# matteocarnelos/microflow-rs

Measured on AMD Instinct MI355X. Metric: inferences/sec (int8) for person_detect.tflite, higher is better.
Workload: dtype i8; 1 GPU; person_detect.tflite batch=65536 per GPU, predict_inner int8->int8, inputs resident in HBM; per_gpu_batch=65536, global_batch=65536, parallelism=batch shard x1, no data-path collective

## Files before the change

microflow_rs_amd/csrc/k_quad.hip:

```cpp
#include "k_common.hpp"

#include <algorithm>
#include <type_traits>

#ifndef MF_QUAD_PRIO
#define MF_QUAD_PRIO 1
#endif
#ifndef MF_Q13_X2A
#define MF_Q13_X2A 0
#define MF_Q13_X2B 0
#define MF_Q57_X2A 3
#define MF_Q57_X2B 3
#endif

#ifndef MF_QUAD_ASM_LDS
#define MF_QUAD_ASM_LDS 0
#endif
#ifndef MF_QUAD_ASM_CLOBBER
#define MF_QUAD_ASM_CLOBBER 1
#endif
#ifndef MF_QUAD_STEM_LDS
#define MF_QUAD_STEM_LDS 1
#endif
#ifndef MF_QUAD_CNT_WAIT
#define MF_QUAD_CNT_WAIT 1
#endif
#ifndef MF_RR_SPARSE
#define MF_RR_SPARSE 0
#endif
#ifndef MF_RR_BLOCK
#define MF_RR_BLOCK 1
#endif
#ifndef MF_RR_SP_PAD
#define MF_RR_SP_PAD 7
#endif
#ifndef MF_Q57_DB
#define MF_Q57_DB 0
#endif
#ifndef MF_QUAD_KO
#define MF_QUAD_KO 0
#endif

namespace mf {
namespace k {
typedef float f32x4 __attribute__((ext_vector_type(4)));

__device__ __forceinline__ void lds_store_asm(uint8_t *p, int off, uint2 v) {
    typedef unsigned int u32x2_ __attribute__((ext_vector_type(2)));
    const uint32_t a = (uint32_t)(uintptr_t)(lds_u8_t *)p;
    const u32x2_ d = {v.x, v.y};
#if MF_QUAD_ASM_CLOBBER
    asm volatile("ds_write_b64 %0, %1 offset:%2" : : "v"(a), "v"(d), "i"(off) : "memory");
#else
    asm volatile("ds_write_b64 %0, %1 offset:%2" : : "v"(a), "v"(d), "i"(off));
#endif
}
__device__ __forceinline__ void lds_store_asm(uint8_t *p, int off, uint4 v) {
    const uint32_t a = (uint32_t)(uintptr_t)(lds_u8_t *)p;
    const u32x4 d = {v.x, v.y, v.z, v.w};
#if MF_QUAD_ASM_CLOBBER
    asm volatile("ds_write_b128 %0, %1 offset:%2" : : "v"(a), "v"(d), "i"(off) : "memory");
#else
    asm volatile("ds_write_b128 %0, %1 offset:%2" : : "v"(a), "v"(d), "i"(off));
#endif
}
template <bool ASMST> __device__ __forceinline__ void quad_barrier() {
    if constexpr (ASMST) asm volatile("s_waitcnt lgkmcnt(0)" ::: "memory");
    wg_sync();
}
__device__ __forceinline__ void quad_barrier_raw() {
    mf_jitter();
    asm volatile("s_waitcnt lgkmcnt(0)\n\ts_barrier" ::: "memory");
    mf_jitter();
}

template <int H_, int W_, int C_, int S_, int N_, int CG_, int CY_, int ORD_, int ROWPAD_, int TS_>
struct RrGeom {
    static constexpr int H = H_, W = W_, C = C_, S = S_, N = N_, CG = CG_, CY = CY_, ORD = ORD_, ROWPAD = ROWPAD_, TS = TS_;
    static constexpr bool PAIR = C == 8;
    static constexpr int OH = (H + S - 1) / S, OW = (W + S - 1) / S, OWC = PAIR ? OW / 2 : OW;
    static constexpr int NQ = PAIR ? 1 : C / 16, CX = 16 / (CG * CY);
    static constexpr int LP = C < 16 ? 16 : C;
    static constexpr int ROWB = W * C, ROW = LP + ROWB + LP + ROWPAD, TILE = (H + 2) * ROW;
    static constexpr int IMG = H * ROWB, ROWCH = ROWB / 16, OPIX = OH * OW;
    static constexpr int NT = (PAIR ? 2 * N : N) / 16, LB = 4 * NT;
    static_assert(C == 8 || C == 16 || C == 32, "register-resident pairs: C <= 32");
    static_assert(CG * CY * CX == 16 && OH % CY == 0 && OWC % CX == 0, "column grid");
    static_assert(ROWB % 16 == 0 && ROWCH <= 64 && ROW % 16 == 0, "staging geometry");
    static_assert(!PAIR || (S == 1 && OW % 2 == 0), "pair columns");
    static_assert(LB == 8 || LB == 16, "one 8- or 16-byte store per lane");
};

template <typename T> struct DstTile {
    static constexpr int TILE = T::TILE, ROW = T::ROW, C = T::C;
};
template <> struct DstTile<void> {
    static constexpr int TILE = 0, ROW = 0, C = 0;
};

template <typename Ge, int G, int NACT, int MG, uint32_t XR4, int X2 = 0>
struct RrPhase {
    static constexpr int NWAVE = NACT;
    static constexpr int UG = G / Ge::CG, UY = Ge::OH / Ge::CY, UX = Ge::OWC / Ge::CX;
    static constexpr int PSY = cgcd(UY, NWAVE), PSX = cgcd(UX, NWAVE / PSY), PSG = cgcd(UG, NWAVE / PSY / PSX);
    static_assert(G % Ge::CG == 0 && PSY * PSX * PSG == NWAVE, "the unit grid does not divide over the waves");
    static constexpr int NUG = UG / PSG, NUY = UY / PSY, NUX = UX / PSX, NU = NUG * NUY * NUX;
    static constexpr int T_UG = Ge::CG * Ge::TILE, T_UY = Ge::CY * Ge::S * Ge::ROW, T_UX = Ge::PAIR ? Ge::CX * 16 : Ge::CX * Ge::S * Ge::C;
    static constexpr int NQ = Ge::NQ, NT = Ge::NT;

    static constexpr bool SP = MF_RR_SPARSE == 1 || (MF_RR_SPARSE == 2 && !Ge::PAIR) || (MF_RR_SPARSE == 3 && Ge::PAIR);
    int tbase[NQ];
    v4i Adw[NQ][3];
    int tb0[NQ], tb1[NQ], tb9[NQ];
    v4i As[NQ];
    int Ai[NQ];
    long A9[NQ];
    float4 dA[NQ], dS[NQ];
    int4 dK[NQ];
    long Apw[NT];
    float4 cA[NT], cS[NT];
    int4 cK[NT];
    int dst_lane;
    int cg, wug;
    float dlo, dhi, plo, phi;

    template <typename NEXT>
    __device__ __forceinline__ void init(const DwPwArgs &p, int lane, int wave) {
        const int col = lane & 15, g = lane >> 4;
        int cy, cx;
        {
            constexpr int ORD = Ge::ORD, CGc = Ge::CG, CYc = Ge::CY, CXc = Ge::CX;
            constexpr int D0 = (ORD == 0 || ORD == 1) ? CGc : (ORD == 2 || ORD == 3) ? CYc : CXc;
            constexpr int D1 = (ORD == 2 || ORD == 4) ? CGc : (ORD == 0 || ORD == 5) ? CYc : CXc;
            const int i0 = col % D0, i1 = (col / D0) % D1, i2 = col / (D0 * D1);
            cg = (ORD == 0 || ORD == 1) ? i0 : (ORD == 2 || ORD == 4) ? i1 : i2;
            cy = (ORD == 2 || ORD == 3) ? i0 : (ORD == 0 || ORD == 5) ? i1 : i2;
            cx = (ORD == 4 || ORD == 5) ? i0 : (ORD == 1 || ORD == 3) ? i1 : i2;
        }
        const int wpy = wave % PSY, wpx = (wave / PSY) % PSX, wpg = wave / (PSY * PSX);
        wug = wpg * Ge::CG;
        const int wave_t = wpg * T_UG + wpy * T_UY + wpx * T_UX;
        auto chunk_addr = [&](int q, int ty, int gch) {
            if constexpr (Ge::PAIR) {
                return cg * Ge::TILE + (cy + ty) * Ge::ROW + Ge::LP + (2 * cx - 2) * 8 + gch * 16 + wave_t;
            } else {
                const int xl = cx * Ge::S + gch - 1;
                return cg * Ge::TILE + (cy * Ge::S + ty) * Ge::ROW + Ge::LP + xl * Ge::C + 16 * (q ^ tile_swz<Ge::TS>(xl)) + wave_t;
            }
        };
#pragma unroll
        for (int q = 0; q < NQ; ++q) {
            tbase[q] = chunk_addr(q, 0, g);
            tb0[q] = g < 3 ? chunk_addr(q, 0, g) : chunk_addr(q, 1, 0);
            tb1[q] = g < 2 ? chunk_addr(q, 1, g + 1) : chunk_addr(q, 2, g - 2);
            tb9[q] = chunk_addr(q, 2, 2) + 8 * (g & 1);
        }
        const int opar = Ge::PAIR ? (g >> 1) : 0;
        const int n0 = Ge::PAIR ? 8 * (g & 1) : (Ge::N / 4) * g;
        const int ox = (Ge::PAIR ? 2 * cx + opar : cx) + wpx * (Ge::PAIR ? 2 : 1) * Ge::CX;
        const int oy = cy + wpy * Ge::CY;
        if constexpr (std::is_void<NEXT>::value) {
            dst_lane = ((cg + wug) * Ge::OPIX + oy * Ge::OW + ox) * Ge::N + n0;
        } else {
            static_assert(NEXT::H == Ge::OH && NEXT::W == Ge::OW && NEXT::C == Ge::N, "the next pair consumes this pair's output");
            static_assert(tile_swz<NEXT::TS>(((Ge::PAIR ? 2 : 1) * Ge::CX) * 255) == 0 || NEXT::TS == 0, "x step vs swizzle");
            const int chunk = n0 >> 4, within = n0 & 15;
            dst_lane = (cg + wug) * NEXT::TILE + (oy + 1) * NEXT::ROW + NEXT::LP + ox * NEXT::C +
                       16 * (NEXT::NQ > 1 ? (chunk ^ tile_swz<NEXT::TS>(ox)) : chunk) + within;
        }
#pragma unroll
        for (int q = 0; q < NQ; ++q) {
            if constexpr (SP) {
                const v4i w0 = ((const v4i *)p.dw.wsp)[(q * 64 + lane) * 2], w1 = ((const v4i *)p.dw.wsp)[(q * 64 + lane) * 2 + 1];
                As[q] = w0, Ai[q] = w1[0];
                A9[q] = (long)(((unsigned long)(uint32_t)w1[2] << 32) | (unsigned long)(uint32_t)w1[1]);
            } else {
#pragma unroll
                for (int ty = 0; ty < 3; ++ty) Adw[q][ty] = ((const v4i *)p.dw.wmm)[(q * 3 + ty) * 64 + lane];
            }
            const int ch4 = Ge::PAIR ? (g & 1) : 4 * q + g;
            dA[q] = ((const float4 *)p.dw.A)[ch4];
            dS[q] = ((const float4 *)p.dw.S)[ch4];
            dK[q] = magic4<MG>(((const int4 *)p.dw.Kc)[ch4]);
        }
#pragma unroll
        for (int m = 0; m < NT; ++m) {
            Apw[m] = ((const long *)p.pw.wrr)[m * 64 + lane];
            cA[m] = *(const float4 *)(p.pw.A + n0 + 4 * m);
            cS[m] = *(const float4 *)(p.pw.S + n0 + 4 * m);
            cK[m] = magic4<MG>(*(const int4 *)(p.pw.Kc + n0 + 4 * m));
        }
        dlo = p.dw.lo_f, dhi = p.dw.hi_f, plo = p.pw.lo_f, phi = p.pw.hi_f;
    }

    template <typename NEXT, bool ASMST = false>
    __device__ __forceinline__ void run(const uint8_t *tb, uint8_t *dst, int gvalid) const {
        constexpr bool TO_LDS = !std::is_void<NEXT>::value;
        constexpr int XF = Ge::PAIR ? 2 : 1;
        constexpr int D_UG = TO_LDS ? Ge::CG * DstTile<NEXT>::TILE : Ge::CG * Ge::OPIX * Ge::N;
        constexpr int D_UY = TO_LDS ? Ge::CY * DstTile<NEXT>::ROW : Ge::CY * Ge::OW * Ge::N;
        constexpr int D_UX = TO_LDS ? XF * Ge::CX * DstTile<NEXT>::C : XF * Ge::CX * Ge::N;
#ifdef MF_QUAD_UB
        constexpr int UB = NU % MF_QUAD_UB == 0 ? MF_QUAD_UB : 1;
#else
        constexpr int UB = NQ > 1 ? 1 : (NU % 2 == 0 ? 2 : 1);
#endif
        auto coords = [](int iu, int &ug, int &uy, int &ux) constexpr {
            ug = (iu / (NUY * NUX)) * PSG, uy = ((iu / NUX) % NUY) * PSY, ux = (iu % NUX) * PSX;
        };
        auto toff_of = [&](int iu) constexpr {
            int ug = 0, uy = 0, ux = 0;
            coords(iu, ug, uy, ux);
            return ug * T_UG + uy * T_UY + ux * T_UX;
        };
        v4i bq[UB][NQ][3], bn[UB][NQ][3];
        long b9[UB][NQ], n9[UB][NQ];
        auto load_taps = [&](v4i (&b)[3], long &e, int q, int toff) {
            if constexpr (SP) {
                b[0] = *(const v4i *)(tb + tb0[q] + toff), b[1] = *(const v4i *)(tb + tb1[q] + toff);
                e = *(const long *)(tb + tb9[q] + toff);
            } else {
#pragma unroll
                for (int ty = 0; ty < 3; ++ty) b[ty] = ((MF_QUAD_KO & 32) && ty > 0) ? b[0] : *(const v4i *)(tb + tbase[q] + toff + ty * Ge::ROW);
            }
        };
#pragma unroll
        for (int u = 0; u < UB; ++u)
#pragma unroll
            for (int q = 0; q < NQ; ++q) load_taps(bq[u][q], b9[u][q], q, toff_of(u));
#pragma unroll
        for (int t0 = 0; t0 < NU; t0 += UB) {
            v4i acc[UB][NQ];
#pragma unroll
            for (int u = 0; u < UB; ++u)
#pragma unroll
                for (int q = 0; q < NQ; ++q) acc[u][q] = v4i{dK[q].x, dK[q].y, dK[q].z, dK[q].w};
#if MF_QUAD_PRIO
            __builtin_amdgcn_s_setprio(MF_QUAD_PRIO);
#endif
            if constexpr (SP) {
                typedef int v8i_ __attribute__((ext_vector_type(8)));
#pragma unroll
                for (int u = 0; u < UB; ++u)
#pragma unroll
                    for (int q = 0; q < NQ; ++q) acc[u][q] = __builtin_amdgcn_mfma_i32_16x16x32_i8(A9[q], b9[u][q], acc[u][q], 0, 0, 0);
                if (t0 + UB < NU) {
#pragma unroll
                    for (int u = 0; u < UB; ++u)
#pragma unroll
                        for (int q = 0; q < NQ; ++q) load_taps(bn[u][q], n9[u][q], q, toff_of(t0 + UB + u));
                }
#pragma unroll
                for (int u = 0; u < UB; ++u)
#pragma unroll
                    for (int q = 0; q < NQ; ++q) {
#if MF_RR_SP_PAD == 11
                        asm volatile("s_nop 11" : "+v"(acc[u][q]));
#else
                        asm volatile("s_nop 7" : "+v"(acc[u][q]));
#endif
                    }
#pragma unroll
                for (int u = 0; u < UB; ++u)
#pragma unroll
                    for (int q = 0; q < NQ; ++q) {
                        const v4i &lo = bq[u][q][0], &hi = bq[u][q][1];
                        const v8i_ B = {lo[0], lo[1], lo[2], lo[3], hi[0], hi[1], hi[2], hi[3]};
                        acc[u][q] = __builtin_amdgcn_smfmac_i32_16x16x128_i8(As[q], B, acc[u][q], Ai[q], 0, 0);
                    }
            } else {
#pragma unroll
                for (int ty = 0; ty < ((MF_QUAD_KO & 256) ? 2 : 3); ++ty)
#pragma unroll
                    for (int u = 0; u < UB; ++u)
#pragma unroll
                        for (int q = 0; q < NQ; ++q)
                            acc[u][q] = __builtin_amdgcn_mfma_i32_16x16x64_i8(Adw[q][ty], bq[u][q][ty], acc[u][q], 0, 0, 0);
            }
#if MF_QUAD_PRIO
            __builtin_amdgcn_s_setprio(0);
#endif
            if (!SP && t0 + UB < NU) {
#pragma unroll
                for (int u = 0; u < UB; ++u)
#pragma unroll
                    for (int q = 0; q < NQ; ++q) load_taps(bn[u][q], n9[u][q], q, toff_of(t0 + UB + u));
            }
#pragma unroll
            for (int u = 0; u < UB; ++u) {
                uint32_t d[2] = {0u, 0u};
                if constexpr ((MF_QUAD_KO & 1) != 0) {
#pragma unroll
                    for (int q = 0; q < NQ; ++q) d[q] = (uint32_t)(acc[u][q][0] ^ acc[u][q][1] ^ acc[u][q][2] ^ acc[u][q][3]);
                } else if constexpr (NQ == 2 && (X2 & 1) != 0) {
                    requant_pack4x2<MG, XR4>(acc[u][0], dA[0], dS[0], acc[u][1], dA[1], dS[1], dlo, dhi, d[0], d[1]);
                } else {
#pragma unroll
                    for (int q = 0; q < NQ; ++q)
                        d[q] = requant_pack4<MG, XR4>(acc[u][q][0], acc[u][q][1], acc[u][q][2], acc[u][q][3], dA[q], dS[q], dlo, dhi);
                }
                const long bop = (long)(((unsigned long)d[1] << 32) | (unsigned long)d[0]);
                uint32_t packed[NT];
                if constexpr ((MF_QUAD_KO & 2) != 0) {
#pragma unroll
                    for (int m = 0; m < NT; ++m) {
                        v4i pa = {cK[m].x, cK[m].y, cK[m].z, cK[m].w};
                        pa = __builtin_amdgcn_mfma_i32_16x16x32_i8(Apw[m], bop, pa, 0, 0, 0);
                        packed[m] = (uint32_t)(pa[0] ^ pa[1] ^ pa[2] ^ pa[3]);
                    }
                } else if constexpr ((X2 & 2) != 0) {
                    static_assert((X2 & 2) == 0 || NT % 2 == 0, "pointwise tiles in pairs");
#pragma unroll
                    for (int m = 0; m < NT; m += 2) {
                        v4i pa = {cK[m].x, cK[m].y, cK[m].z, cK[m].w}, pb2 = {cK[m + 1].x, cK[m + 1].y, cK[m + 1].z, cK[m + 1].w};
                        pa = __builtin_amdgcn_mfma_i32_16x16x32_i8(Apw[m], bop, pa, 0, 0, 0);
                        pb2 = __builtin_amdgcn_mfma_i32_16x16x32_i8(Apw[m + 1], bop, pb2, 0, 0, 0);
                        requant_pack4x2<MG, XR4>(pa, cA[m], cS[m], pb2, cA[m + 1], cS[m + 1], plo, phi, packed[m], packed[m + 1]);
                    }
                } else {
#pragma unroll
                    for (int m = 0; m < NT; ++m) {
                        v4i pa = {cK[m].x, cK[m].y, cK[m].z, cK[m].w};
                        pa = __builtin_amdgcn_mfma_i32_16x16x32_i8(Apw[m], bop, pa, 0, 0, 0);
                        packed[m] = requant_pack4<MG, XR4>(pa[0], pa[1], pa[2], pa[3], cA[m], cS[m], plo, phi);
                    }
                }
                int ug = 0, uy = 0, ux = 0;
                coords(t0 + u, ug, uy, ux);
                const int doff = ug * D_UG + uy * D_UY + ux * D_UX;
                if (G == 1 || cg + wug + ug * Ge::CG < gvalid) {
                    if constexpr (TO_LDS && ASMST) {
                        static_assert(G * DstTile<NEXT>::TILE < 65536, "tile offsets fit the ds offset field");
                        if constexpr (Ge::LB == 8) lds_store_asm(dst + dst_lane, doff, make_uint2(packed[0], packed[1]));
                        else lds_store_asm(dst + dst_lane, doff, make_uint4(packed[0], packed[1], packed[2], packed[3]));
                    } else if constexpr (TO_LDS) {
                        if constexpr (Ge::LB == 8) *(uint2 *)(dst + dst_lane + doff) = make_uint2(packed[0], packed[1]);
                        else *(uint4 *)(dst + dst_lane + doff) = make_uint4(packed[0], packed[1], packed[2], packed[3]);
                    } else if (!(MF_QUAD_KO & 4) || packed[0] == 0x12345678u) {
                        if constexpr (Ge::LB == 8) st_out(dst + dst_lane + doff, make_uint2(packed[0], packed[1]));
                        else st_out(dst + dst_lane + doff, make_uint4(packed[0], packed[1], packed[2], packed[3]));
                    }
                }
            }
#pragma unroll
            for (int u = 0; u < UB; ++u)
#pragma unroll
                for (int q = 0; q < NQ; ++q) {
#pragma unroll
                    for (int ty = 0; ty < 3; ++ty) bq[u][q][ty] = bn[u][q][ty];
                    b9[u][q] = n9[u][q];
                }
        }
    }
};

template <typename Ge, int NWAVE_, int MG, uint32_t XR4>
struct BlkPhase {
    static constexpr int NWAVE = NWAVE_, NU = Ge::W / 16;
    static constexpr int LP = 4, ROW = 320, PLANE = (Ge::H + 2) * ROW, BYTES = 2 * PLANE;
    static_assert(Ge::C == 8 && Ge::S == 1 && Ge::N == 16 && Ge::CG == 1, "block form: 8 -> 16 channels, stride 1, one image per step");
    static_assert(Ge::H == 4 * NWAVE && Ge::W % 16 == 0, "two block rows per wave, whole units per row");
    static_assert(ROW >= 4 * Ge::W + 2 * LP && ROW % 256 == 64 && BYTES % 16 == 0 && PLANE + 64 * NU + 8 < 65536, "tile A planes");
    int tbase;
    int dst_lane;
    v4i Adw[2];
    long Apw[4];
    float4 dA[2], dS[2], cA, cS;
    int4 dK[2], cK;
    float dlo, dhi, plo, phi;

    template <typename NEXT>
    __device__ __forceinline__ void init(const DwPwArgs &p, int lane, int wave) {
        static_assert(NEXT::H == Ge::OH && NEXT::W == Ge::OW && NEXT::C == Ge::N && NEXT::NQ == 1, "pair B consumes this pair's output, unswizzled");
        const int n = lane & 15, g = lane >> 4, by = 2 * wave + (n >> 3), bcx = n & 7;
        tbase = (2 * by + g) * ROW + 8 * bcx;
        dst_lane = (2 * by + 1) * NEXT::ROW + NEXT::LP + 32 * bcx + 4 * g;
#pragma unroll
        for (int q = 0; q < 2; ++q) {
            Adw[q] = ((const v4i *)p.dw.wblk)[q * 64 + lane];
            dA[q] = ((const float4 *)p.dw.A)[q];
            dS[q] = ((const float4 *)p.dw.S)[q];
            dK[q] = magic4<MG>(((const int4 *)p.dw.Kc)[q]);
        }
#pragma unroll
        for (int s = 0; s < 4; ++s) Apw[s] = ((const long *)p.pw.wiso)[s * 64 + lane];
        cA = *(const float4 *)(p.pw.A + 4 * g);
        cS = *(const float4 *)(p.pw.S + 4 * g);
        cK = magic4<MG>(*(const int4 *)(p.pw.Kc + 4 * g));
        dlo = p.dw.lo_f, dhi = p.dw.hi_f, plo = p.pw.lo_f, phi = p.pw.hi_f;
    }

    template <typename NEXT, bool ASMST = false>
    __device__ __forceinline__ void run(const uint8_t *tb, uint8_t *dst, int) const {
        static_assert(!ASMST, "the block form stores with plain LDS stores");
        typedef unsigned int u32x2_ __attribute__((ext_vector_type(2)));
        typedef __attribute__((address_space(3))) const volatile u32x2_ lds_cv2;
        v4i b[NU][2];
#pragma unroll
        for (int u = 0; u < NU; ++u)
#pragma unroll
            for (int q = 0; q < 2; ++q) {
                lds_u8_t *a = (lds_u8_t *)(tb + tbase) + (q * PLANE + 64 * u);
                const u32x2_ lo = *(lds_cv2 *)a, hi = *(lds_cv2 *)(a + 8);
                b[u][q] = v4i{(int)lo[0], (int)lo[1], (int)hi[0], (int)hi[1]};
            }
#pragma unroll
        for (int u = 0; u < NU; ++u) {
            v4i acc[2];
#if MF_QUAD_PRIO
            __builtin_amdgcn_s_setprio(MF_QUAD_PRIO);
#endif
#pragma unroll
            for (int q = 0; q < 2; ++q)
                acc[q] = __builtin_amdgcn_mfma_i32_16x16x64_i8(Adw[q], b[u][q], v4i{dK[q].x, dK[q].y, dK[q].z, dK[q].w}, 0, 0, 0);
#if MF_QUAD_PRIO
            __builtin_amdgcn_s_setprio(0);
#endif
            uint32_t d[2];
#pragma unroll
            for (int q = 0; q < 2; ++q) d[q] = requant_pack4<MG, XR4>(acc[q][0], acc[q][1], acc[q][2], acc[q][3], dA[q], dS[q], dlo, dhi);
            const long bop = (long)(((unsigned long)d[1] << 32) | (unsigned long)d[0]);
#pragma unroll
            for (int s = 0; s < 4; ++s) {
                const v4i pa = __builtin_amdgcn_mfma_i32_16x16x32_i8(Apw[s], bop, v4i{cK.x, cK.y, cK.z, cK.w}, 0, 0, 0);
                *(uint32_t *)(dst + dst_lane + 256 * u + (s >> 1) * NEXT::ROW + (s & 1) * 16) =
                    requant_pack4<MG, XR4>(pa[0], pa[1], pa[2], pa[3], cA, cS, plo, phi);
            }
        }
    }
};


#ifndef MF_Q13B_ROWPAD
#define MF_Q13B_ROWPAD 32
#endif
#ifndef MF_Q13A_ROWPAD
#define MF_Q13A_ROWPAD 32
#endif
struct Quad13 {
    using A = RrGeom<48, 48, 8, 1, 16, 1, 4, 0, MF_Q13A_ROWPAD, 0x000>;
    using B = RrGeom<48, 48, 16, 2, 32, 1, 2, 0, MF_Q13B_ROWPAD, 0x000>;
    static constexpr int G = 1, NTHR = 768, WPE = 3, ACT_A = 12, ACT_B = 12, X2A = MF_Q13_X2A, X2B = MF_Q13_X2B;
    static constexpr bool DBA = false;
    static constexpr const char *name = "quad_rr<48,48,8,1,16|48,48,16,2,32>";
};
struct Quad57 {
    using A = RrGeom<24, 24, 32, 1, 32, 1, 2, 0, 0, 0x002>;
    using B = RrGeom<24, 24, 32, 2, 64, 1, 4, 0, 32, 0x002>;
    static constexpr int G = 1, NTHR = 256, WPE = 2, ACT_A = 4, ACT_B = 3, X2A = MF_Q57_X2A, X2B = MF_Q57_X2B;
    static constexpr bool DBA = MF_Q57_DB != 0;
    static constexpr const char *name = "quad_rr<24,24,32,1,32|24,24,32,2,64>";
};



template <typename P, typename = void> struct blk_or {
    static constexpr int ROW = 0, LP = 0, PLANE = 0;
};
template <typename P> struct blk_or<P, std::void_t<decltype(P::PLANE)>> {
    static constexpr int ROW = P::ROW, LP = P::LP, PLANE = P::PLANE;
};
template <typename Q, bool STEM> constexpr bool quad_blk() {
    return STEM && MF_RR_BLOCK != 0 && MF_QUAD_ASM_LDS == 0;
}
template <typename Q, bool STEM, int MG, uint32_t XR4>
using QuadPhaseA = std::conditional_t<quad_blk<Q, STEM>(), BlkPhase<typename Q::A, Q::ACT_A, MG, XR4>, RrPhase<typename Q::A, Q::G, Q::ACT_A, MG, XR4, Q::X2A>>;
template <typename Q, bool STEM> constexpr int quad_buf_a() {
    if constexpr (quad_blk<Q, STEM>()) return BlkPhase<typename Q::A, Q::ACT_A, 1, 0u>::BYTES;
    else return Q::G * Q::A::TILE;
}
template <typename Q, bool STEM> constexpr int quad_stem_bytes() {
    return STEM ? 16 + (2 * Q::A::H + 2) * (2 * Q::A::W) : 0;
}
template <typename Q, bool STEM, int MG, uint32_t XR4, bool F32IN = false>
__global__ __launch_bounds__(Q::NTHR, Q::WPE) void quad_rr(const int8_t *__restrict__ in, int8_t *__restrict__ out, QuadArgs p, int batch) {
    static_assert(!F32IN || STEM, "the f32 entry is the stem's");
    using GA = typename Q::A;
    using GB = typename Q::B;
    epi_enter<MG>();
    constexpr int G = Q::G, NTHR = Q::NTHR, NWAVE = NTHR / 64;
    constexpr bool DBA = Q::DBA && !STEM;
    constexpr bool BLK = quad_blk<Q, STEM>();
    constexpr int BUF_A = quad_buf_a<Q, STEM>(), OFF_B = (DBA ? 2 : 1) * BUF_A + 512, BUF_B = G * GB::TILE, OFF_S = OFF_B + BUF_B + 512;
    constexpr int S_GUARD = 16, SW = 2 * GA::W, SH = 2 * GA::H, S_TILE = quad_stem_bytes<Q, STEM>(), OFF_Q = OFF_S + S_TILE;
    constexpr int OFF_F = OFF_Q + 16;
    constexpr int OFF_C = OFF_F + (F32IN ? 4 * SH * SW : 0);
    constexpr bool ASMST = MF_QUAD_ASM_LDS == 2 || (MF_QUAD_ASM_LDS == 1 && STEM);
    constexpr bool STEM_LDS = STEM && MF_QUAD_STEM_LDS != 0 && ((!F32IN && MG == 3) || MF_QUAD_STEM_LDS > 1);
    static_assert(!STEM || (G == 1 && GA::C == 8 && GA::W == 48 && (GA::H / 2) % NWAVE == 0 && (SH * SW) % 1024 == 0 && S_TILE % 16 == 0),
                  "stem phase: 8 channels, 24 pixel pairs per output row, whole row pairs per wave");
    extern __shared__ __attribute__((aligned(16))) uint8_t lds[];
    const int tid = threadIdx.x, lane = tid & 63;
    const int wave = __builtin_amdgcn_readfirstlane(tid >> 6);
    DynSteps dq;
    dq.init(lds + OFF_Q, p.a.dw.queue, tid, p.a.dw.qcfg);
    if constexpr (STEM)
        for (int i = tid; i < S_TILE / 16; i += NTHR) ((uint4 *)(lds + OFF_S))[i] = make_uint4(p.stem_izp4, p.stem_izp4, p.stem_izp4, p.stem_izp4);
    if constexpr (STEM_LDS)
        if (tid < 152) ((uint32_t *)(lds + OFF_C))[tid] = p.stem[tid] + ((MG != 0 && tid >= 144) ? (uint32_t)MF_MAGIC_I : 0u);
    for (int i = tid; i < OFF_B / 16; i += NTHR) ((uint4 *)lds)[i] = make_uint4(p.a.dw.izp4, p.a.dw.izp4, p.a.dw.izp4, p.a.dw.izp4);
    for (int i = tid; i < (BUF_B + 512) / 16; i += NTHR) ((uint4 *)(lds + OFF_B))[i] = make_uint4(p.b.dw.izp4, p.b.dw.izp4, p.b.dw.izp4, p.b.dw.izp4);
    QuadPhaseA<Q, STEM, MG, XR4> pa;
    RrPhase<GB, G, Q::ACT_B, MG, XR4, Q::X2B> pb;
    pa.template init<GB>(p.a, lane, wave);
    pb.template init<void>(p.b, lane, wave);
    wg_sync();

    auto stage = [&](int st, int buf = 0) {
        if constexpr (F32IN) {
            constexpr int NI = SH * SW * 4 / 1024;
            static_assert(NI % NWAVE == 0, "f32 staging: whole pieces per wave");
#pragma unroll
            for (int k = 0; k < NI / NWAVE; ++k) {
                const int r = k * NWAVE + wave;
                dma16(in + ((size_t)st * (SH * SW * 4) + r * 1024 + lane * 16), lds + OFF_F + r * 1024);
            }
            return;
        }
        if constexpr (STEM) {
            constexpr int NI = SH * SW / 1024;
#pragma unroll
            for (int k = 0; k < (NI + NWAVE - 1) / NWAVE; ++k) {
                const int r = k * NWAVE + wave;
                if (r < NI) dma16(in + ((size_t)st * (SH * SW) + r * 1024 + lane * 16), lds + OFF_S + S_GUARD + SW + r * 1024);
            }
            return;
        }
        constexpr int NROWS = G * GA::H;
        const int src_lane = GA::NQ > 1 ? (lane ^ tile_swz<GA::TS>(lane / (GA::NQ > 1 ? GA::NQ : 1))) : lane;
#pragma unroll
        for (int k = 0; k < (NROWS + NWAVE - 1) / NWAVE; ++k) {
            const int r = k * NWAVE + wave;
            const int gi = r / GA::H, y = r % GA::H;
            if (r < NROWS && st * G + gi < batch && lane < GA::ROWCH)
                dma16(in + ((size_t)(st * G + gi) * GA::IMG + y * GA::ROWB + src_lane * 16), lds + buf * BUF_A + gi * GA::TILE + (y + 1) * GA::ROW + GA::LP);
        }
    };
    auto quant_rows = [&]() {
        if constexpr (F32IN && !(MF_QUAD_KO & 64)) {
            constexpr int RPW = GA::H / 2 / NWAVE, NR = 4 * RPW + 1, C4 = SW / 4, NIT = (NR * C4 + 63) / 64;
            asm volatile("" ::: "memory");
            if constexpr (MG == 3) __builtin_amdgcn_s_setreg(0x801, 0);
            asm volatile("" ::: "memory");
            const int y0 = 4 * RPW * wave - 1;
#pragma unroll
            for (int it = 0; it < NIT; ++it) {
                const int item = it * 64 + lane, row = item / C4, c4 = item - row * C4, y = y0 + row;
                if (item < NR * C4 && y >= 0) {
                    const f32x4 v = *(const f32x4 *)(lds + OFF_F + (y * SW + 4 * c4) * 4);
                    int qv[4];
                    float q[4];
                    bool plain = p.in_fast != 0;
#pragma unroll
                    for (int e = 0; e < 4; ++e) {
                        const float q0 = __fmul_rn(v[e], p.in_rcp);
                        q[e] = __fmaf_rn(__fmaf_rn(-p.in_scale, q0, v[e]), p.in_rcp, q0);
                        plain = plain && (__builtin_fabsf(q[e]) <= 3.0e38f);
                    }
                    if constexpr ((MF_QUAD_KO & 128) != 0) {
#pragma unroll
                        for (int e = 0; e < 4; ++e) qv[e] = __float_as_int(v[e]);
                    } else if (__builtin_expect(plain, 1)) {
#pragma unroll
                        for (int e = 0; e < 4; ++e) {
                            const float t = __fadd_rn(q[e], p.in_zp_f);
                            const float r = __fadd_rn(t, __builtin_copysignf(0x1.fffffep-2f, t));
                            qv[e] = (int)__builtin_amdgcn_fmed3f(r, p.in_sat_lo, p.in_sat_hi);
                        }
                    } else {
#pragma unroll
                        for (int e = 0; e < 4; ++e) {
                            const float t = __fadd_rn(__fdiv_rn(v[e], p.in_scale), p.in_zp_f);
                            const float r = __fadd_rn(t, __builtin_copysignf(0x1.fffffep-2f, t));
                            qv[e] = (r != r) ? 0 : (int)__builtin_amdgcn_fmed3f(r, p.in_sat_lo, p.in_sat_hi);
                        }
                    }
                    *(uint32_t *)(lds + OFF_S + S_GUARD + (y + 1) * SW + 4 * c4) = pack4(qv[0], qv[1], qv[2], qv[3]) ^ p.in_xr4;
                }
            }
            asm volatile("" ::: "memory");
            if constexpr (MG == 3) __builtin_amdgcn_s_setreg(0x801, 3);
            asm volatile("" ::: "memory");
        }
    };
    auto stem_phase = [&](const uint32_t *sc) {
        constexpr int RPW = GA::H / 2 / NWAVE;
        const int col = lane & 15, g = lane >> 4;
        const int cq = (g & 1) * 4;
        long Aw;
        v4i cA_, cS_, cK;
        if constexpr (STEM_LDS) {
            const uint32_t *lsc = (const uint32_t *)(lds + OFF_C);
            Aw = *(const long *)(lsc + 2 * lane);
            cA_ = *(const v4i *)(lsc + 128 + cq), cS_ = *(const v4i *)(lsc + 136 + cq), cK = *(const v4i *)(lsc + 144 + cq);
        } else {
            typedef __attribute__((address_space(1))) const uint32_t g_u32;
            g_u32 *gsc = (g_u32 *)(uintptr_t)sc;
            typedef long i64x1 __attribute__((ext_vector_type(1)));
            Aw = (*(__attribute__((address_space(1))) const i64x1 *)(gsc + 2 * lane))[0];
            cA_ = *(__attribute__((address_space(1))) const v4i *)(gsc + 128 + cq), cS_ = *(__attribute__((address_space(1))) const v4i *)(gsc + 136 + cq);
            const v4i ck_ = *(__attribute__((address_space(1))) const v4i *)(gsc + 144 + cq);
            const int4 ck = magic4<MG>(make_int4(ck_[0], ck_[1], ck_[2], ck_[3]));
            cK = v4i{ck.x, ck.y, ck.z, ck.w};
        }
        const float4 cA = make_float4(__int_as_float(cA_[0]), __int_as_float(cA_[1]), __int_as_float(cA_[2]), __int_as_float(cA_[3]));
        const float4 cS = make_float4(__int_as_float(cS_[0]), __int_as_float(cS_[1]), __int_as_float(cS_[2]), __int_as_float(cS_[3]));
        const int oy1 = col >= 8 ? 1 : 0, j1 = col >= 8 ? col - 8 : 16 + col;
        const int off0 = S_GUARD + g * SW + 4 * col - 4, off1 = S_GUARD + (2 * oy1 + g) * SW + 4 * j1 - 4, off2 = S_GUARD + (2 + g) * SW + 4 * (8 + col) - 4;
        using PA = QuadPhaseA<Q, STEM, MG, XR4>;
        constexpr int A_ROW = BLK ? blk_or<PA>::ROW : GA::ROW, A_LP = BLK ? blk_or<PA>::LP : GA::LP, A_PX = BLK ? 8 : 16;
        const int px = BLK ? (g & 1) * blk_or<PA>::PLANE + (g >> 1) * 4 : (g >> 1) * 8 + cq;
        const int dst0 = A_ROW + A_LP + A_PX * col + px, dst1 = (1 + oy1) * A_ROW + A_LP + A_PX * j1 + px, dst2 = 2 * A_ROW + A_LP + A_PX * (8 + col) + px;
#pragma unroll
        for (int i = 0; i < RPW; ++i) {
            const int rp = wave * RPW + i;
            const uint8_t *t0 = lds + OFF_S + rp * (4 * SW);
            uint8_t *d0 = lds + rp * (2 * A_ROW);
            long B[3];
#pragma unroll
            for (int n = 0; n < 3; ++n) {
                const uint32_t *q = (const uint32_t *)(t0 + (n == 0 ? off0 : (n == 1 ? off1 : off2)));
                uint32_t lo = q[0];
                const uint32_t hi = q[1];
                if (n == 0) lo = col == 0 ? p.stem_izp4 : lo;
                if (n == 1) lo = col == 8 ? p.stem_izp4 : lo;
                B[n] = (long)(((unsigned long)hi << 32) | (unsigned long)lo);
            }
#pragma unroll
            for (int n = 0; n < 3; ++n) {
                const v4i acc = __builtin_amdgcn_mfma_i32_16x16x32_i8(Aw, B[n], cK, 0, 0, 0);
                *(uint32_t *)(d0 + (n == 0 ? dst0 : (n == 1 ? dst1 : dst2))) =
                    requant_pack4<MG, XR4>(acc[0], acc[1], acc[2], acc[3], cA, cS, p.stem_lo, p.stem_hi);
            }
        }
    };
    const int nsteps = (batch + G - 1) / G;
    if (dq.step < nsteps) stage(dq.step);
    int ko_steps = 0;
    const uint32_t *sc = p.stem;
    if constexpr (STEM) {
        asm volatile("s_waitcnt vmcnt(0)" ::: "memory");
        wg_sync();
        if (dq.step < nsteps) quant_rows(), stem_phase(sc);
        for (; dq.step < nsteps; dq.advance(tid)) {
            const int step = dq.step;
            if (!(MF_QUAD_KO & 16)) quad_barrier<ASMST>();
            dq.top(tid);
            if (dq.nxt < nsteps && !((MF_QUAD_KO & 8) && ko_steps > 0)) stage(dq.nxt);
            if (Q::ACT_A == NWAVE || wave < Q::ACT_A) pa.template run<GB, ASMST>(lds, lds + OFF_B, 1);
            asm volatile("s_waitcnt vmcnt(0)" ::: "memory");
            if (!(MF_QUAD_KO & 16)) quad_barrier<ASMST>();
            if (Q::ACT_B == NWAVE || wave < Q::ACT_B)
                pb.template run<void>(lds + OFF_B, (uint8_t *)out + (size_t)step * GB::OPIX * GB::N, 1);
            asm volatile("" : "+s"(sc));
            if (dq.nxt < nsteps) quant_rows(), stem_phase(sc);
            ++ko_steps;
        }
    } else {
        bool first = true;
        int cur = 0;
        for (; dq.step < nsteps; dq.advance(tid)) {
            const int step = dq.step;
            if (MF_QUAD_CNT_WAIT && G == 1 && !first && (Q::ACT_B == NWAVE || wave < Q::ACT_B)) {
                constexpr int NSTORE = decltype(pb)::NU;
                static_assert(NSTORE >= 0 && NSTORE < 16, "counted wait");
                asm volatile("s_waitcnt vmcnt(%0)" ::"n"(NSTORE) : "memory");
            } else {
                asm volatile("s_waitcnt vmcnt(0)" ::: "memory");
            }
            first = false;
            if constexpr (MF_QUAD_CNT_WAIT != 0 && G == 1) quad_barrier_raw();
            else quad_barrier<ASMST>();
            dq.top(tid);
            const int gvalid = min(G, batch - step * G);
            if constexpr (DBA) {
                if (dq.nxt < nsteps && !((MF_QUAD_KO & 8) && ko_steps > 0)) stage(dq.nxt, cur ^ 1);
            }
            if (Q::ACT_A == NWAVE || wave < Q::ACT_A) pa.template run<GB, ASMST>(lds + (DBA ? cur * BUF_A : 0), lds + OFF_B, gvalid);
            if (!(MF_QUAD_KO & 16)) quad_barrier<ASMST>();
            if constexpr (!DBA) {
                if (dq.nxt < nsteps && !((MF_QUAD_KO & 8) && ko_steps > 0)) stage(dq.nxt);
            }
            if (Q::ACT_B == NWAVE || wave < Q::ACT_B)
                pb.template run<void>(lds + OFF_B, (uint8_t *)out + (size_t)step * G * GB::OPIX * GB::N, gvalid);
            cur ^= 1;
            ++ko_steps;
        }
    }
    dq.finish(tid);
}

template <typename Q, bool STEM, int MG, uint32_t XR4, bool F32IN = false>
static void launch_quad_t(const int8_t *in, int8_t *out, const QuadArgs &a, int batch, hipStream_t s) {
    constexpr int lds = ((Q::DBA && !STEM) ? 2 : 1) * quad_buf_a<Q, STEM>() + 512 + Q::G * Q::B::TILE + 512 + quad_stem_bytes<Q, STEM>() + 16 +
                        (F32IN ? 4 * (2 * Q::A::H) * (2 * Q::A::W) : 0) + (STEM ? 640 : 0);
    static_assert(lds <= 163840, "quad tiles do not fit the LDS");
    static LaunchState st;
    const int per_cu = prepared(st, quad_rr<Q, STEM, MG, XR4, F32IN>, Q::NTHR, lds);
    const int nsteps = (batch + Q::G - 1) / Q::G;
    const int grid = nsteps < 256 * per_cu ? nsteps : 256 * per_cu;
    QuadArgs b = a;
    using GA = typename Q::A;
    using GB = typename Q::B;
    const double hbm = (double)batch * ((STEM ? (F32IN ? 16 : 4) * GA::H * GA::W : GA::H * GA::W * GA::C) + GB::OPIX * GB::N);
    const double rq = (double)batch * ((STEM ? GA::H * GA::W * GA::C : 0) + GA::OPIX * (GA::C + GA::N) + GB::OPIX * (GB::C + GB::N));
    b.a.dw.qcfg = dq_config(nsteps, grid, dq_est_us(hbm, rq));
    b.a.dw.queue = dq_slot(b.a.dw.queue, b.a.dw.qlaunch);
    MF_LAUNCH((quad_rr<Q, STEM, MG, XR4, F32IN>), dim3(grid), dim3(Q::NTHR), lds, s, in, out, b, batch);
}
template <typename Q> static bool quad_matches(int H, int W, int C, int S, int N, int H2, int W2, int C2, int S2, int N2) {
    using GA = typename Q::A;
    using GB = typename Q::B;
    return H == GA::H && W == GA::W && C == GA::C && S == GA::S && N == GA::N && H2 == GB::H && W2 == GB::W && C2 == GB::C && S2 == GB::S &&
           N2 == GB::N;
}
static int quad_mask() {
    const int m = switches().quads;
    return m;
}
const char *quad_name(int H, int W, int C, int S, int N, int H2, int W2, int C2, int S2, int N2) {
    if ((quad_mask() & 1) && quad_matches<Quad13>(H, W, C, S, N, H2, W2, C2, S2, N2)) return Quad13::name;
    if ((quad_mask() & 2) && quad_matches<Quad57>(H, W, C, S, N, H2, W2, C2, S2, N2)) return Quad57::name;
    return nullptr;
}
const char *quad_stem_name(int SH, int SW, int H, int W, int C, int S, int N, int H2, int W2, int C2, int S2, int N2) {
    if ((quad_mask() & 4) && SH == 2 * Quad13::A::H && SW == 2 * Quad13::A::W && quad_matches<Quad13>(H, W, C, S, N, H2, W2, C2, S2, N2))
        return "penta_rr<96,96,1,2,8|48,48,8,1,16|48,48,16,2,32>";
    return nullptr;
}
bool launch_quad(int H, int W, int C, int S, int N, int H2, int W2, int C2, int S2, int N2, const int8_t *in, int8_t *out, const QuadArgs &a,
                 int batch, hipStream_t s) {
    if (!a.a.dw.wmm || !a.a.pw.wrr || !a.b.dw.wmm || !a.b.pw.wrr) return false;
    if (MF_RR_SPARSE && (!a.a.dw.wsp || !a.b.dw.wsp)) return false;
    if (a.stem && quad_blk<Quad13, true>() && (!a.a.dw.wblk || !a.a.pw.wiso)) return false;
    int mg = std::min(std::min(a.a.dw.magic, a.a.pw.magic), std::min(a.b.dw.magic, a.b.pw.magic));
    if (a.stem) mg = std::min(mg, a.stem_magic);
    if (mg == 0) return false;
#define MF_QUAD_GO2(Q, ST)                                                                         \
    do {                                                                                           \
        if (mg == 3) {                                                                             \
            launch_quad_t<Q, ST, 3, 0u>(in, out, a, batch, s);                                     \
        } else if (a.b.pw.xr) {                                                                           \
            if (mg == 2) launch_quad_t<Q, ST, 2, 0x80808080u>(in, out, a, batch, s);               \
            else launch_quad_t<Q, ST, 1, 0x80808080u>(in, out, a, batch, s);                       \
        } else {                                                                                   \
            if (mg == 2) launch_quad_t<Q, ST, 2, 0u>(in, out, a, batch, s);                        \
            else launch_quad_t<Q, ST, 1, 0u>(in, out, a, batch, s);                                \
        }                                                                                          \
        return true;                                                                               \
    } while (0)
#define MF_QUAD_GO(Q) MF_QUAD_GO2(Q, false)
    if (quad_matches<Quad13>(H, W, C, S, N, H2, W2, C2, S2, N2)) {
        if (a.stem) MF_QUAD_GO2(Quad13, true);
        MF_QUAD_GO(Quad13);
    }
    if (quad_matches<Quad57>(H, W, C, S, N, H2, W2, C2, S2, N2)) {
        MF_QUAD_GO(Quad57);
    }
#undef MF_QUAD_GO
#undef MF_QUAD_GO2
    return false;
}
bool launch_quad_f32(int H, int W, int C, int S, int N, int H2, int W2, int C2, int S2, int N2, const float *in, int8_t *out, const QuadArgs &a,
                     int batch, hipStream_t s) {
    if (!a.stem || !a.f32_ok || !(quad_mask() & 4) || !quad_matches<Quad13>(H, W, C, S, N, H2, W2, C2, S2, N2)) return false;
    if (!a.a.dw.wmm || !a.a.pw.wrr || !a.b.dw.wmm || !a.b.pw.wrr) return false;
    if (MF_RR_SPARSE && (!a.a.dw.wsp || !a.b.dw.wsp)) return false;
    if (quad_blk<Quad13, true>() && (!a.a.dw.wblk || !a.a.pw.wiso)) return false;
    const int mg = std::min(std::min(std::min(a.a.dw.magic, a.a.pw.magic), std::min(a.b.dw.magic, a.b.pw.magic)), a.stem_magic);
    if (mg == 0) return false;
    const int8_t *src = (const int8_t *)in;
    if (mg == 3) launch_quad_t<Quad13, true, 3, 0u, true>(src, out, a, batch, s);
    else if (a.b.pw.xr) {
        if (mg == 2) launch_quad_t<Quad13, true, 2, 0x80808080u, true>(src, out, a, batch, s);
        else launch_quad_t<Quad13, true, 1, 0x80808080u, true>(src, out, a, batch, s);
    } else {
        if (mg == 2) launch_quad_t<Quad13, true, 2, 0u, true>(src, out, a, batch, s);
        else launch_quad_t<Quad13, true, 1, 0u, true>(src, out, a, batch, s);
    }
    return true;
}

}
}
```

Baseline: 30.83 million inferences/s.

## Add block-form depthwise/pointwise phase for the 24x24x32 quad kernel

Adds a Blk32Phase that runs the first dw+pw pair of the ops 5..8 quad kernel in two stages. Depthwise MFMAs over 8x8 pixel units write int8 results to a new swizzled LDS mid buffer, then a pointwise pass reads from it after a barrier. The stage of the next image is issued between the two stages so it overlaps the pointwise work. This replaces the RrPhase path and aims to use all four waves with better LDS access patterns. The cost is an extra barrier and a larger LDS footprint, which is checked to stay within two workgroups per CU. The path requires the wblk weights and falls back otherwise.

```diff
diff --git a/microflow_rs_amd/csrc/k_quad.hip b/microflow_rs_amd/csrc/k_quad.hip
--- a/microflow_rs_amd/csrc/k_quad.hip
+++ b/microflow_rs_amd/csrc/k_quad.hip
@@ -30,6 +30,9 @@
 #endif
 #ifndef MF_RR_BLOCK
 #define MF_RR_BLOCK 1
+#endif
+#ifndef MF_Q57_BLOCK
+#define MF_Q57_BLOCK 1
 #endif
 #ifndef MF_RR_SP_PAD
 #define MF_RR_SP_PAD 7
@@ -430,6 +433,148 @@
     }
 };
 
+template <typename Ge, int NWAVE_, int MG, uint32_t XR4, int X2>
+struct Blk32Phase {
+    static constexpr int NWAVE = NWAVE_;
+    static constexpr int LP = 32, ROW = LP + Ge::ROWB, TILE = (Ge::H + 2) * ROW + 32;
+    static constexpr int MROW = Ge::ROWB + 16, MID = Ge::H * MROW;
+    static constexpr int UX = Ge::W / 8, NU = (Ge::H / 8) * UX;
+    static constexpr int RPW = Ge::H / 2 / NWAVE, NPW = RPW * UX;
+    static_assert(Ge::C == 32 && Ge::N == 32 && Ge::S == 1 && Ge::CG == 1 && NWAVE == 4, "block form: 32 -> 32 channels, stride 1, two quads per wave");
+    static_assert(Ge::H % 8 == 0 && Ge::W % 8 == 0 && (Ge::H / 2) % NWAVE == 0, "whole units, whole row pairs per wave");
+    static_assert(ROW % 256 == 32 && MROW % 256 == 16 && TILE % 16 == 0 && MID % 16 == 0 && Ge::ROWCH <= 64, "tile A and MID pitches");
+    static_assert((Ge::H / 8) * 8 * ROW + UX * 256 + 128 < 65536 && Ge::H * MROW < 65536, "unit offsets fit the ds offset field");
+    __host__ __device__ static constexpr int swz(int tile_row) { return (tile_row >> 2) & 1; }
+    __host__ __device__ static constexpr int mid_f(int x, int y) { return ((x >> 2) & 1) | (((y >> 2) & 1) << 1); }
+    int tbase;
+    int mid_st;
+    int mid_ld[RPW];
+    int dst_lane;
+    v4i Adw[2];
+    long Apw[2];
+    float4 dA[2], dS[2], cA[2], cS[2];
+    int4 dK[2], cK[2];
+    float dlo, dhi, plo, phi;
+
+    template <typename NEXT>
+    __device__ __forceinline__ void init(const DwPwArgs &p, int lane, int wave) {
+        static_assert(NEXT::H == Ge::OH && NEXT::W == Ge::OW && NEXT::C == Ge::N && NEXT::NQ == 2, "pair B consumes this pair's output");
+        static_assert(tile_swz<NEXT::TS>(8 * 255) == 0, "x step of a pixel group vs tile B's swizzle");
+        const int n = lane & 15, g = lane >> 4;
+        {
+            const int by = n >> 2, bx = n & 3, r = 2 * by + g;
+            tbase = r * ROW + 64 * bx + 16 * ((wave >> 1) ^ swz(r)) + 8 * (wave & 1);
+            const int y = 2 * by + (g >> 1), x = 2 * bx + (g & 1);
+            mid_st = y * MROW + 32 * x + 8 * (wave ^ mid_f(x, y));
+        }
+        {
+            const int yy = n >> 3, x = n & 7;
+#pragma unroll
+            for (int rp = 0; rp < RPW; ++rp) {
+                const int y = 2 * (RPW * wave + rp) + yy;
+                mid_ld[rp] = y * MROW + 32 * x + 8 * (g ^ mid_f(x, y));
+            }
+            dst_lane = (2 * RPW * wave + yy + 1) * NEXT::ROW + NEXT::LP + x * NEXT::C + 16 * ((g >> 1) ^ tile_swz<NEXT::TS>(x)) + 8 * (g & 1);
+        }
+#pragma unroll
+        for (int q = 0; q < 2; ++q) {
+            const int ch4 = 2 * wave + q;
+            Adw[q] = ((const v4i *)p.dw.wblk)[ch4 * 64 + lane];
+            dA[q] = ((const float4 *)p.dw.A)[ch4];
+            dS[q] = ((const float4 *)p.dw.S)[ch4];
+            dK[q] = magic4<MG>(((const int4 *)p.dw.Kc)[ch4]);
+        }
+        const int n0 = 8 * g;
+#pragma unroll
+        for (int m = 0; m < 2; ++m) {
+            const long w = ((const long *)p.pw.wrr)[m * 64 + lane];
+            const int wlo = (int)(uint32_t)(unsigned long)w, whi = (int)(uint32_t)((unsigned long)w >> 32);
+            const int sa = 4 * (n + 16 * ((2 * g) & 3)), sb = 4 * (n + 16 * ((2 * g + 1) & 3));
+            const int alo = __builtin_amdgcn_ds_bpermute(sa, wlo), ahi = __builtin_amdgcn_ds_bpermute(sa, whi);
+            const int blo = __builtin_amdgcn_ds_bpermute(sb, wlo), bhi = __builtin_amdgcn_ds_bpermute(sb, whi);
+            const uint32_t lo = (uint32_t)(g < 2 ? alo : ahi), hi = (uint32_t)(g < 2 ? blo : bhi);
+            Apw[m] = (long)(((unsigned long)hi << 32) | (unsigned long)lo);
+            cA[m] = *(const float4 *)(p.pw.A + n0 + 4 * m);
+            cS[m] = *(const float4 *)(p.pw.S + n0 + 4 * m);
+            cK[m] = magic4<MG>(*(const int4 *)(p.pw.Kc + n0 + 4 * m));
+        }
+        dlo = p.dw.lo_f, dhi = p.dw.hi_f, plo = p.pw.lo_f, phi = p.pw.hi_f;
+    }
+
+    __device__ __forceinline__ void run_dw(const uint8_t *tb, uint8_t *mid) const {
+        typedef unsigned int u32x2_ __attribute__((ext_vector_type(2)));
+        typedef __attribute__((address_space(3))) const volatile u32x2_ lds_c2;
+        typedef __attribute__((address_space(3))) u32x2_ lds_2;
+        auto load = [&](u32x2_(&b)[4], int u) {
+            lds_u8_t *a = (lds_u8_t *)(tb + tbase) + ((u / UX) * 8 * ROW + (u % UX) * 256);
+#pragma unroll
+            for (int xx = 0; xx < 4; ++xx) b[xx] = *(lds_c2 *)(a + 32 * xx);
+        };
+        auto taps = [&](u32x2_(&b)[4], v4i(&acc)[2]) {
+            uint32_t a1 = b[0][1], b0 = b[1][0], c1 = b[2][1], d0 = b[3][0];
+            asm("v_swap_b32 %0, %1" : "+v"(a1), "+v"(b0));
+            asm("v_swap_b32 %0, %1" : "+v"(c1), "+v"(d0));
+            const v4i X = {(int)b[0][0], (int)a1, (int)b[2][0], (int)c1}, Y = {(int)b0, (int)b[1][1], (int)d0, (int)b[3][1]};
+#if MF_QUAD_PRIO
+            __builtin_amdgcn_s_setprio(MF_QUAD_PRIO);
+#endif
+            acc[0] = __builtin_amdgcn_mfma_i32_16x16x64_i8(Adw[0], X, v4i{dK[0].x, dK[0].y, dK[0].z, dK[0].w}, 0, 0, 0);
+            acc[1] = __builtin_amdgcn_mfma_i32_16x16x64_i8(Adw[1], Y, v4i{dK[1].x, dK[1].y, dK[1].z, dK[1].w}, 0, 0, 0);
+#if MF_QUAD_PRIO
+            __builtin_amdgcn_s_setprio(0);
+#endif
+        };
+        u32x2_ b1[4], b2[4];
+        v4i acc[2], accn[2];
+        load(b1, 0);
+        if (NU > 1) load(b2, 1);
+        taps(b1, acc);
+#pragma unroll
+        for (int u = 0; u < NU; ++u) {
+#pragma unroll
+            for (int xx = 0; xx < 4; ++xx) b1[xx] = b2[xx];
+            if (u + 2 < NU) load(b2, u + 2);
+            if (u + 1 < NU) taps(b1, accn);
+            uint32_t d[2];
+            if constexpr ((X2 & 1) != 0) {
+                requant_pack4x2<MG, XR4>(acc[0], dA[0], dS[0], acc[1], dA[1], dS[1], dlo, dhi, d[0], d[1]);
+            } else {
+#pragma unroll
+                for (int q = 0; q < 2; ++q) d[q] = requant_pack4<MG, XR4>(acc[q][0], acc[q][1], acc[q][2], acc[q][3], dA[q], dS[q], dlo, dhi);
+            }
+            *(lds_2 *)((lds_u8_t *)(mid + mid_st) + ((u / UX) * 8 * MROW + (u % UX) * 256)) = u32x2_{d[0], d[1]};
+            acc[0] = accn[0], acc[1] = accn[1];
+        }
+    }
+
+    template <typename NEXT>
+    __device__ __forceinline__ void run_pw(const uint8_t *mid, uint8_t *dst) const {
+        typedef unsigned int u32x2_ __attribute__((ext_vector_type(2)));
+        typedef __attribute__((address_space(3))) const volatile u32x2_ lds_c2;
+        typedef __attribute__((address_space(3))) u32x2_ lds_2;
+        long b[NPW];
+#pragma unroll
+        for (int j = 0; j < NPW; ++j) {
+            const u32x2_ v = *(lds_c2 *)((lds_u8_t *)(mid + mid_ld[j / UX]) + (j % UX) * 256);
+            b[j] = (long)(((unsigned long)v[1] << 32) | (unsigned long)v[0]);
+        }
+#pragma unroll
+        for (int j = 0; j < NPW; ++j) {
+            v4i pa = {cK[0].x, cK[0].y, cK[0].z, cK[0].w}, pb = {cK[1].x, cK[1].y, cK[1].z, cK[1].w};
+            pa = __builtin_amdgcn_mfma_i32_16x16x32_i8(Apw[0], b[j], pa, 0, 0, 0);
+            pb = __builtin_amdgcn_mfma_i32_16x16x32_i8(Apw[1], b[j], pb, 0, 0, 0);
+            uint32_t o[2];
+            if constexpr ((X2 & 2) != 0) {
+                requant_pack4x2<MG, XR4>(pa, cA[0], cS[0], pb, cA[1], cS[1], plo, phi, o[0], o[1]);
+            } else {
+                o[0] = requant_pack4<MG, XR4>(pa[0], pa[1], pa[2], pa[3], cA[0], cS[0], plo, phi);
+                o[1] = requant_pack4<MG, XR4>(pb[0], pb[1], pb[2], pb[3], cA[1], cS[1], plo, phi);
+            }
+            *(lds_2 *)((lds_u8_t *)(dst + dst_lane) + ((j / UX) * 2 * NEXT::ROW + (j % UX) * 8 * NEXT::C)) = u32x2_{o[0], o[1]};
+        }
+    }
+};
+
 
 #ifndef MF_Q13B_ROWPAD
 #define MF_Q13B_ROWPAD 32
@@ -463,11 +608,22 @@
 template <typename Q, bool STEM> constexpr bool quad_blk() {
     return STEM && MF_RR_BLOCK != 0 && MF_QUAD_ASM_LDS == 0;
 }
+template <typename Q, bool STEM> constexpr bool quad_blk32() {
+    return !STEM && MF_Q57_BLOCK != 0 && MF_QUAD_ASM_LDS == 0 && !Q::DBA && Q::G == 1 && Q::A::C == 32 && Q::A::N == 32 && Q::A::S == 1 && Q::ACT_A == 4 &&
+           Q::NTHR == 256;
+}
 template <typename Q, bool STEM, int MG, uint32_t XR4>
-using QuadPhaseA = std::conditional_t<quad_blk<Q, STEM>(), BlkPhase<typename Q::A, Q::ACT_A, MG, XR4>, RrPhase<typename Q::A, Q::G, Q::ACT_A, MG, XR4, Q::X2A>>;
+using QuadPhaseA = std::conditional_t<quad_blk<Q, STEM>(), BlkPhase<typename Q::A, Q::ACT_A, MG, XR4>,
+                                      std::conditional_t<quad_blk32<Q, STEM>(), Blk32Phase<typename Q::A, 4, MG, XR4, Q::X2A>,
+                                                         RrPhase<typename Q::A, Q::G, Q::ACT_A, MG, XR4, Q::X2A>>>;
 template <typename Q, bool STEM> constexpr int quad_buf_a() {
     if constexpr (quad_blk<Q, STEM>()) return BlkPhase<typename Q::A, Q::ACT_A, 1, 0u>::BYTES;
+    else if constexpr (quad_blk32<Q, STEM>()) return Blk32Phase<typename Q::A, 4, 1, 0u, 0>::TILE;
     else return Q::G * Q::A::TILE;
+}
+template <typename Q, bool STEM> constexpr int quad_mid_bytes() {
+    if constexpr (quad_blk32<Q, STEM>()) return Blk32Phase<typename Q::A, 4, 1, 0u, 0>::MID;
+    else return 0;
 }
 template <typename Q, bool STEM> constexpr int quad_stem_bytes() {
     return STEM ? 16 + (2 * Q::A::H + 2) * (2 * Q::A::W) : 0;
@@ -485,6 +641,9 @@
     constexpr int S_GUARD = 16, SW = 2 * GA::W, SH = 2 * GA::H, S_TILE = quad_stem_bytes<Q, STEM>(), OFF_Q = OFF_S + S_TILE;
     constexpr int OFF_F = OFF_Q + 16;
     constexpr int OFF_C = OFF_F + (F32IN ? 4 * SH * SW : 0);
+    constexpr bool BLK32 = quad_blk32<Q, STEM>();
+    constexpr int OFF_M = OFF_C + (STEM ? 640 : 0);
+    static_assert(!BLK32 || (OFF_M % 16 == 0 && OFF_M + quad_mid_bytes<Q, STEM>() <= 80 * 1024), "two workgroups per CU");
     constexpr bool ASMST = MF_QUAD_ASM_LDS == 2 || (MF_QUAD_ASM_LDS == 1 && STEM);
     constexpr bool STEM_LDS = STEM && MF_QUAD_STEM_LDS != 0 && ((!F32IN && MG == 3) || MF_QUAD_STEM_LDS > 1);
     static_assert(!STEM || (G == 1 && GA::C == 8 && GA::W == 48 && (GA::H / 2) % NWAVE == 0 && (SH * SW) % 1024 == 0 && S_TILE % 16 == 0),
@@ -523,6 +682,17 @@
             for (int k = 0; k < (NI + NWAVE - 1) / NWAVE; ++k) {
                 const int r = k * NWAVE + wave;
                 if (r < NI) dma16(in + ((size_t)st * (SH * SW) + r * 1024 + lane * 16), lds + OFF_S + S_GUARD + SW + r * 1024);
+            }
+            return;
+        }
+        if constexpr (BLK32) {
+            using PA = QuadPhaseA<Q, STEM, MG, XR4>;
+            static_assert(GA::H % NWAVE == 0, "whole rows per wave");
+#pragma unroll
+            for (int k = 0; k < GA::H / NWAVE; ++k) {
+                const int y = k * NWAVE + wave;
+                if (st < batch && lane < GA::ROWCH)
+                    dma16(in + ((size_t)st * GA::IMG + y * GA::ROWB + (lane ^ PA::swz(y + 1)) * 16), lds + (y + 1) * PA::ROW + PA::LP);
             }
             return;
         }
@@ -676,10 +846,18 @@
             if constexpr (DBA) {
                 if (dq.nxt < nsteps && !((MF_QUAD_KO & 8) && ko_steps > 0)) stage(dq.nxt, cur ^ 1);
             }
-            if (Q::ACT_A == NWAVE || wave < Q::ACT_A) pa.template run<GB, ASMST>(lds + (DBA ? cur * BUF_A : 0), lds + OFF_B, gvalid);
-            if (!(MF_QUAD_KO & 16)) quad_barrier<ASMST>();
-            if constexpr (!DBA) {
+            if constexpr (BLK32) {
+                pa.run_dw(lds, lds + OFF_M);
+                if (!(MF_QUAD_KO & 16)) quad_barrier<ASMST>();
                 if (dq.nxt < nsteps && !((MF_QUAD_KO & 8) && ko_steps > 0)) stage(dq.nxt);
+                pa.template run_pw<GB>(lds + OFF_M, lds + OFF_B);
+                if (!(MF_QUAD_KO & 16)) quad_barrier<ASMST>();
+            } else {
+                if (Q::ACT_A == NWAVE || wave < Q::ACT_A) pa.template run<GB, ASMST>(lds + (DBA ? cur * BUF_A : 0), lds + OFF_B, gvalid);
+                if (!(MF_QUAD_KO & 16)) quad_barrier<ASMST>();
+                if constexpr (!DBA) {
+                    if (dq.nxt < nsteps && !((MF_QUAD_KO & 8) && ko_steps > 0)) stage(dq.nxt);
+                }
             }
             if (Q::ACT_B == NWAVE || wave < Q::ACT_B)
                 pb.template run<void>(lds + OFF_B, (uint8_t *)out + (size_t)step * G * GB::OPIX * GB::N, gvalid);
@@ -693,8 +871,9 @@
 template <typename Q, bool STEM, int MG, uint32_t XR4, bool F32IN = false>
 static void launch_quad_t(const int8_t *in, int8_t *out, const QuadArgs &a, int batch, hipStream_t s) {
     constexpr int lds = ((Q::DBA && !STEM) ? 2 : 1) * quad_buf_a<Q, STEM>() + 512 + Q::G * Q::B::TILE + 512 + quad_stem_bytes<Q, STEM>() + 16 +
-                        (F32IN ? 4 * (2 * Q::A::H) * (2 * Q::A::W) : 0) + (STEM ? 640 : 0);
+                        (F32IN ? 4 * (2 * Q::A::H) * (2 * Q::A::W) : 0) + (STEM ? 640 : 0) + quad_mid_bytes<Q, STEM>();
     static_assert(lds <= 163840, "quad tiles do not fit the LDS");
+    static_assert(!quad_blk32<Q, STEM>() || lds <= 80 * 1024, "the block form of ops 5..8 keeps two workgroups per CU");
     static LaunchState st;
     const int per_cu = prepared(st, quad_rr<Q, STEM, MG, XR4, F32IN>, Q::NTHR, lds);
     const int nsteps = (batch + Q::G - 1) / Q::G;
@@ -733,6 +912,7 @@
     if (!a.a.dw.wmm || !a.a.pw.wrr || !a.b.dw.wmm || !a.b.pw.wrr) return false;
     if (MF_RR_SPARSE && (!a.a.dw.wsp || !a.b.dw.wsp)) return false;
     if (a.stem && quad_blk<Quad13, true>() && (!a.a.dw.wblk || !a.a.pw.wiso)) return false;
+    if (!a.stem && quad_blk32<Quad57, false>() && quad_matches<Quad57>(H, W, C, S, N, H2, W2, C2, S2, N2) && !a.a.dw.wblk) return false;
     int mg = std::min(std::min(a.a.dw.magic, a.a.pw.magic), std::min(a.b.dw.magic, a.b.pw.magic));
     if (a.stem) mg = std::min(mg, a.stem_magic);
     if (mg == 0) return false;
```

Measured after the change: 31.43 million inferences/s (median of 6 runs). 1.9% higher.
